# cvlab-stonybrook/s-volsdf

Hardware: AMD Instinct MI355X
Metric: rendered rays/sec (1024-ray batch, 128 samples) (higher is better)
Workload: dtype f32 (every product, forward and backward, as three fp16 MFMA products of two-piece fp16 operands with f32 accumulate; activation blocks hold both pieces: float32 accuracy class)

## Files before the change

include/svolsdf_hip.h:

```cpp
#ifndef SVOLSDF_HIP_H
#define SVOLSDF_HIP_H

#include <stddef.h>
#include <stdint.h>

#ifdef __cplusplus
extern "C" {
#endif

int svs_version(void);
const char* svs_last_error_string(void);

int svs_set_deterministic(int on);
int svs_get_deterministic(void);

int svs_rays_from_uv(const float* uv, const float* pose, const float* intrinsics, int n_rays, float* ray_dirs,
                     float* cam_loc, float* depth_scale, void* hip_stream);

int svs_eikonal_points(const float* uniform_points, const float* cam_loc, const float* z_eik, const float* ray_dirs,
                       int n_rays, float* points, void* hip_stream);
int svs_stage_in(const void* pinned_host, void* device, size_t bytes, void* hip_stream);
int svs_split_last(const float* z, int n_rays, int n, float* head, float* last, void* hip_stream);

enum { SVS_MMA_F32 = 0, SVS_MMA_F16X2 = 1, SVS_MMA_F16X2_HALF = 2 };
// ... 74 lines not shown
  const float* absmax;
  const float *rec0, *rec1;
} svs_wgrad_job;
int svs_wgrad_multi(const svs_wgrad_job* jobs, int n_jobs, int precision, void* hip_stream);
int svs_wgrad(const float* a0, const float* b0, long long sa0, long long sb0, const float* a1, const float* b1,
              long long sa1, long long sb1, const float* b_extra, long long s_extra, int n_points, int precision,
              const float* absmax, const float* rec0, const float* rec1, float* dW, int ldw, float* db, void* hip_stream);

size_t svs_block_bytes(int n_points, int blocks_per_tile);
size_t svs_rgb_zbuf_bytes(int n_points);
size_t svs_sdf_ubuf_bytes(int n_points);
size_t svs_sdf_gbuf_bytes(int n_points);
int svs_rgb_bwd(int n_points, const float* d_rgb, const float* rgb, const float* rbuf, const float* stream, int precision,
                float* zbuf, float* feat_bar, float* d_normals, float* absmax, void* hip_stream);
int svs_sdf_bwd_a(const float* points, int n_points, const float* cam, int cam_stride, const float* dirs, const float* z,
                  int S, int n_rays, const float* d_grad, const unsigned char* clamp_mask, const float* hbuf,
                  const float* gbuf, const float* stream, int precision, float* ubuf, float* a2buf, float* pebuf,
                  float* absmax, void* hip_stream);
int svs_sdf_bwd_b(int n_points, const float* d_sdf, const unsigned char* clamp_mask, const float* feat_bar,
                  int n_feat_points, const float* hbuf, const float* gbuf, const float* a2buf, const float* ubuf,
                  const float* stream, int precision, float* abuf, float* sbar_out, float* absmax, void* hip_stream);
int svs_lin8_row0_grad(const float* hbuf, const float* ubuf, const float* sbar, int n_points, int precision, float* out257,
                       void* hip_stream);
int svs_unpack_wgrad(const float* dWk, const float* dbk, int ldw, int map, int rows, int cols, int row_off,
                     const float* weight_v, const float* weight_g, const float* row0, float* grad_v, float* grad_g,
                     float* grad_b, void* hip_stream);
typedef struct svs_unpack_job {
  const float *dWk, *dbk;
  int ldw, map, rows, cols, row_off;
  const float *weight_v, *weight_g, *row0;
  float *grad_v, *grad_g, *grad_b;
} svs_unpack_job;
int svs_unpack_wgrad_multi(const svs_unpack_job* jobs, int n_jobs, void* hip_stream);

size_t svs_adam_workspace_bytes(void);
int svs_clip_guard_adam(float* params, float* grads, float* exp_avg, float* exp_avg_sq, long long n, int step,
                        int* step_counter, double max_norm, double lr, double beta1, double beta2, double eps,
                        void* workspace, float* info, void* hip_stream);

int svs_cost_lookup(const float* xyz, const float* cam, const float* dirs, const float* z, int S, int n_points,
                    int n_views, int same_view, int inverse_depth, float img_w, float img_h, const float* view_params,
                    const float* const* cost, const float* const* z_near, const float* const* z_far, const int* dims,
                    float* pj, float* pi, unsigned char* valid, const int* same_view_dev, void* hip_stream);

int svs_loss(int n_rays, int n_samples, int n_eik, const float* rgb_values, const float* rgb_target,
             const float* grad_theta, const float* weights, const float* pi, const float* pj, const float* depth_values,
// ... 108 lines not shown
```

s-volsdf_amd/csrc/svs_mlp_bwd.hip:

```cpp
#include "svs_mlp_dev.h"
#include "svs_mlp_bwd_args.h"
#include "svs_ticket.h"

namespace svs {
namespace mlp {


__global__ __launch_bounds__(kThreads, 1) void rgb_bwd_kernel(RgbBwdArgs a) {
  extern __shared__ __attribute__((aligned(16))) unsigned char smem[];
  Stream st;
  st.g = a.stream; st.buf = reinterpret_cast<f32x4*>(smem); st.cur = 1;
  const int lane = threadIdx.x & 63, half = lane >> 5, wave = threadIdx.x >> 6;
  const int wtile = blockIdx.x * kWaves + wave;
  const int p = wtile * kTilePts + (lane & 31);
  const bool livep = p < a.P;
  const int pc = livep ? p : a.P - 1;
  const size_t LS = block_stride();
  const float* rb = a.rbuf + (size_t)wtile * kBlockF;
  float* zb = a.zbuf + (size_t)wtile * kBlockF;

  st.prefetch<kW4TF4>();
  float dz[3];
#pragma unroll
  for (int c = 0; c < 3; ++c) {
// ... 403 lines not shown
  SdfBwdAArgs a;
  const bool h2 = is_h2(precision);
  if (n_points < 0 || n_rays < 0 || (n_points == 0 && n_rays == 0) || (n_points > 0 && !points) ||
      (n_rays > 0 && !(cam && dirs && z && S > 0)) || !d_grad || !hbuf || (!h2 && !gbuf) || !stream || !ubuf || (!h2 && !a2buf) ||
      !pebuf) {
    set_error("svs_sdf_bwd_a: null/invalid argument"); return SVS_EINVAL;
  }
  a.src.pts = points; a.src.cam = cam; a.src.dirs = dirs; a.src.z = z; a.src.cam_stride = cam_stride;
  a.src.S = S > 0 ? S : 1; a.src.n_ray = n_rays * (S > 0 ? S : 0); a.src.P = a.src.n_ray + n_points;
  a.d_grad = d_grad; a.clamp_mask = clamp_mask; a.hbuf = hbuf; a.gbuf = gbuf;
  a.stream = reinterpret_cast<const f32x4*>(stream); a.ubuf = ubuf; a.a2buf = a2buf; a.pebuf = pebuf;
  a.absmax = absmax;
  if (h2) {
    if (!absmax) { set_error("svs_sdf_bwd_a: fp16x2 needs absmax"); return SVS_EINVAL; }
    return launch_sdf_bwd_a_h2(a, precision == kFmtF16x2, (hipStream_t)hip_stream);
  }
  if (precision != kFmtF32) { set_error("svs_sdf_bwd_a: unknown precision %d", precision); return SVS_EINVAL; }
  static int once = set_lds_b(sdf_bwd_a_kernel, kLdsBytes, "svs_sdf_bwd_a");
  if (once) return once;
  sdf_bwd_a_kernel<<<(a.src.P + kWgPts - 1) / kWgPts, kThreads, kLdsBytes, (hipStream_t)hip_stream>>>(a);
  return check_launch("svs_sdf_bwd_a");
}

int svs_sdf_bwd_b(int n_points, const float* d_sdf, const unsigned char* clamp_mask, const float* feat_bar,
                  int n_feat_points, const float* hbuf, const float* gbuf, const float* a2buf, const float* ubuf,
                  const float* stream, int precision, float* abuf, float* sbar_out, float* absmax, void* hip_stream) {
  const bool h2 = is_h2(precision);
  if (!hbuf || !gbuf || (h2 ? !ubuf : !a2buf) || !stream || !abuf || !sbar_out || n_points <= 0 || n_feat_points % 32) {
    set_error("svs_sdf_bwd_b: null/invalid argument (n_feat_points must be a multiple of 32)"); return SVS_EINVAL;
  }
  SdfBwdBArgs a{n_points, d_sdf, clamp_mask, feat_bar, n_feat_points / 32, hbuf, gbuf, a2buf, ubuf,
                reinterpret_cast<const f32x4*>(stream) + kSdfTrainPassBF4, abuf, sbar_out, absmax,
                gbuf + 7 * (size_t)tiles_of(n_points) * kBlockF, (size_t)kBlockF};
  if (h2) {
    if (!absmax) { set_error("svs_sdf_bwd_b: fp16x2 needs absmax"); return SVS_EINVAL; }
    return launch_sdf_bwd_b_h2(a, precision == kFmtF16x2, (hipStream_t)hip_stream);
  }
  if (precision != kFmtF32) { set_error("svs_sdf_bwd_b: unknown precision %d", precision); return SVS_EINVAL; }
  static int once = set_lds_b(sdf_bwd_b_kernel, kLdsBytes, "svs_sdf_bwd_b");
  if (once) return once;
  sdf_bwd_b_kernel<<<(n_points + kWgPts - 1) / kWgPts, kThreads, kLdsBytes, (hipStream_t)hip_stream>>>(a);
  return check_launch("svs_sdf_bwd_b");
}

int svs_lin8_row0_grad(const float* hbuf, const float* ubuf, const float* sbar, int n_points, int precision, float* out257,
                       void* hip_stream) {
  if (!hbuf || !sbar || !out257 || n_points <= 0) { set_error("svs_lin8_row0_grad: bad argument"); return SVS_EINVAL; }
  if (is_h2(precision)) return launch_lin8_row0_h2(hbuf, ubuf, sbar, n_points, tiles_of(n_points), out257, precision == kFmtF16x2, (hipStream_t)hip_stream);
  if (precision != kFmtF32) { set_error("svs_lin8_row0_grad: unknown precision %d", precision); return SVS_EINVAL; }
  const int n_tiles = (n_points + 31) / 32;
  const int grid = n_tiles < 1024 ? n_tiles : 1024;
  const det::Ticket ticket{det::take_slots(1), 0u, (unsigned)grid};
  lin8_row0_kernel<<<grid, 256, 0, (hipStream_t)hip_stream>>>(hbuf, ubuf, sbar, n_tiles, tiles_of(n_points), n_points, out257, ticket);
  return check_launch("svs_lin8_row0_grad");
}

int svs_unpack_wgrad(const float* dWk, const float* dbk, int ldw, int map, int rows, int cols, int row_off,
                     const float* weight_v, const float* weight_g, const float* row0, float* grad_v, float* grad_g,
                     float* grad_b, void* hip_stream) {
  if (!dWk || !weight_v || !grad_v || rows < 1 || cols < 1 || map < 0 || map > 4 || (weight_g && !grad_g)) {
    set_error("svs_unpack_wgrad: bad argument"); return SVS_EINVAL;
  }
  UnpackArgs a{dWk, dbk, ldw, map, rows, cols, row_off, weight_v, weight_g, grad_v, grad_g, grad_b, row0};
  unpack_wgrad_kernel<<<(rows + 3) / 4, 256, 0, (hipStream_t)hip_stream>>>(a);
  return check_launch("svs_unpack_wgrad");
// ... 23 lines not shown
```

s-volsdf_amd/csrc/svs_mlp_bwd_args.h:

```cpp
#pragma once
#include "svs_mlp_dev.h"

namespace svs {
namespace mlp {

struct RgbBwdArgs {
  int P;
  const float* d_rgb;
  const float* rgb;
  const float* rbuf;
  const f32x4* stream;
  float* zbuf;
  float* feat_bar;
  float* d_normals;
  float* absmax;
};
constexpr int kRbufFb = 4 * kBlockF + 1024;

struct SdfBwdAArgs {
  PointSrc src;
  const float* d_grad;
  const unsigned char* clamp_mask;
  const float* hbuf;
  const float* gbuf;
  const f32x4* stream;
  float* ubuf;
  float* a2buf;
  float* pebuf;
  float* absmax;
};

struct SdfBwdBArgs {
  int P;
  const float* d_sdf;
  const unsigned char* clamp_mask;
  const float* feat_bar;
  int n_feat_tiles;
  const float* hbuf; const float* gbuf;
  const float* a2buf;
  const float* ubuf;
  const f32x4* stream;
  float* abuf;
  float* sbar_out;
  float* absmax;
  const float* w0; size_t w0_stride;
  int reverse = 0;
};
int launch_bg_bwd_b_h2(const SdfBwdBArgs& a, bool gp, hipStream_t s);

int launch_rgb_bwd_h2(const RgbBwdArgs& a, bool gp, hipStream_t s);
int launch_lin8_row0_h2(const float* hbuf, const float* ubuf, const float* sbar, int n_points, int n_tiles_pad, float* out257,
                        bool gp, hipStream_t s);
int launch_sdf_bwd_a_h2(const SdfBwdAArgs& a, bool gp, hipStream_t s);
int launch_sdf_bwd_b_h2(const SdfBwdBArgs& a, bool gp, hipStream_t s);

}
}
```

s-volsdf_amd/csrc/svs_mlp_bwd_h2.hip:

```cpp
#include "svs_mlp_h2_dev.h"
#include "svs_mlp_host.h"
#include "svs_mlp_bwd_args.h"
#include "svs_mlp_h2_trunk.h"
#include "svs_mlp_bwd_h2_dev.h"
#include "svs_ticket.h"
#include <cstdlib>

namespace svs {
namespace mlp {

template <bool GP>
struct RgbBwdEpi {
  f32x16 prev;
  TilePieces r;
  float v8[8];
  Pieces2* out;
  float* zblk;
  PointScale* ps;
  int lane;
  __device__ __forceinline__ void b(int tp, int rr) {
    float v = prev[rr] * ps->inv_in;
    v = hi_at(r, rr) > 0.0f ? v : 0.0f;
    pin(v);
    ps->track(v);
// ... 321 lines not shown
      st.advance();
    }
    ep.all(7);
    ep.end();
    ps.next();
  }
  for (int l = 1; l < 7; ++l) {
    PassAEpi<true, GP> ep;
    ep.out = &pa; ep.ublk = ub + (size_t)(l + 1) * LS; ep.urec = urec(l + 1);
    ep.ps = &ps; ep.splice = splice; ep.lane = lane; ep.half = half; ep.l3 = l == 3;
    pass_a_layer_h2<true, false, GP>(st, pb, ep, hb + (size_t)l * LS, lane);
#pragma unroll
    for (int s = 0; s < 16; ++s) { pb.h[s] = pa.h[s]; pb.m[s] = pa.m[s]; }
  }
  {
    PassAEpi<false, GP> ep;
    ep.out = nullptr; ep.ublk = ub + (size_t)8 * LS; ep.urec = urec(8);
    ep.ps = &ps; ep.splice = splice; ep.lane = lane; ep.half = half; ep.l3 = false;
    pass_a_layer_h2<false, true, GP>(st, pb, ep, hb + (size_t)7 * LS, lane);
  }
  publish_max(a.absmax, ps.gmax);
}

template <bool FIRST, bool SPLIT, typename Net, bool A2, bool GP>
struct PassBEpi {
  static constexpr bool kG = A2 || FIRST;
  f32x16 prev;
  TilePieces h, u, g;
  float v, s1, q;
  float v8[8];
  f16x8 ap[2], aq[2];
  Pieces2* out;
  float* ablk;
  float* arec;
  PointScale* ps;
  float sbar, u_inv100;
  int lane, half;
  bool l4;
  __device__ __forceinline__ void a(int r) {
    v = prev[r] * ps->inv_in;
    float e = __builtin_amdgcn_exp2f(grad_times<GP>(h, r, -100.0f * 1.44269504088896341f));
    if (A2) e = __builtin_fminf(e, 0.99999994f);
    s1 = 1.0f - e;
    if (A2) q = e * u_inv100;
    pin(v); pin(s1);
    if (A2) pin(q);
  }
  template <bool LATE = false>
  __device__ __forceinline__ void b(int tp, int r) {
    float o = v * s1;
    if (A2) {
      const float gg = grad_mix<GP>(g, r);
      const float t = grad_times<GP>(u, r, gg);
      o = __builtin_fmaf(t, q * __builtin_amdgcn_rcpf(s1), o);
      if (FIRST) o = __builtin_fmaf(sbar, gg, o);
    } else if (FIRST) {
      o = __builtin_fmaf(sbar, grad_mix<GP>(g, r), o);
    }
    if (l4 && tp > Net::kSpliceTile) o = 0.0f;
    if (l4 && tp == Net::kSpliceTile) {
      const bool z0 = rho(r) >= Net::kSpliceLocal, z1 = rho(r) + 4 >= Net::kSpliceLocal;
      if (z0 || z1) { if (half ? z1 : z0) o = 0.0f; }
    }
    pin(o);
    ps->track(o);
    v8[r & 7] = o * ps->s_out;
    if ((r & 7) == 7) {
      const int k = 2 * tp + (r >> 3), q2 = r >> 3;
      if (SPLIT) {
        split8(v8, out->h[k], out->m[k]);
        pin(out->h[k], out->m[k]);
        ap[q2] = out->h[k];
        if (GP) aq[q2] = out->m[k];
      } else if (GP) {
        split8(v8, ap[q2], aq[q2]);
      } else {
        ap[q2] = hi8(v8, 1.0f);
      }
      if (!LATE) store_grad<GP>(ablk, k, lane, ap[q2], aq[q2]);
    }
  }
  __device__ __forceinline__ void store_slot(int tp, int s) {
    if (s == 9) store_grad<GP>(ablk, 2 * tp, lane, ap[0], aq[0]);
    if (s == 15) store_grad<GP>(ablk, 2 * tp + 1, lane, ap[1], aq[1]);
  }
  __device__ __forceinline__ void all(int tp) {
#pragma unroll
    for (int r = 0; r < 16; ++r) { a(r); b(tp, r); }
  }
};

template <bool FIRST, bool SPLIT, bool LAST_STAGE, typename Net, bool A2, bool GP>
__device__ __forceinline__ void pass_b_stage_h2(Stream& st, const Pieces2& in, PassBEpi<FIRST, SPLIT, Net, A2, GP>& ep, const float* hblk,
                                                const float* ublk, const float* urec, const float* gblk, float next_floor, int lane) {
  constexpr bool kG = A2 || FIRST;
  store_record(ep.arec, lane, ep.ps->s_out, 0.0f);
  ep.u_inv100 = A2 ? 100.0f * PointScale::inv_pow2(load_scale(urec, lane)) : 0.0f;
  TilePieces hnext, unext, gnext;
  load_tile_grad<GP>(hblk, 0, lane, hnext);
  if (A2) load_tile_grad<GP>(ublk, 0, lane, unext);
  if (kG) load_tile_grad<GP>(gblk, 0, lane, gnext);
  constexpr int kPer = GP ? 4 : 2;
  constexpr int kLoads = kPer * (1 + (A2 ? 1 : 0) + (kG ? 1 : 0));
  constexpr int kStores = GP ? 4 : 2;
#pragma unroll
  for (int t = 0; t < 8; ++t) {
    const TilePieces hcur = hnext, ucur = unext, gcur = gnext;
    auto side = [&](int s) {
      if (t == 7) return;
      if (s == 10) hnext.h[0] = load_piece(hblk, 2 * (t + 1), lane);
      if (s == 11) hnext.h[1] = load_piece(hblk, 2 * (t + 1) + 1, lane);
      if (A2 && s == 12) unext.h[0] = load_piece(ublk, 2 * (t + 1), lane);
      if (A2 && s == 13) unext.h[1] = load_piece(ublk, 2 * (t + 1) + 1, lane);
      if (kG && s == 14) gnext.h[0] = load_piece(gblk, 2 * (t + 1), lane);
      if (kG && s == 15) gnext.h[1] = load_piece(gblk, 2 * (t + 1) + 1, lane);
      if (GP) {
// ... 5 lines not shown
        if (kG && s == 15) gnext.m[1] = load_piece(gblk, 2 * (t + 1) + 1, lane, 1);
      }
    };
    const bool fetch = !(LAST_STAGE && t == 7);
    f32x16 acc;
    if (!fetch) acc = tile_mma_h2<16>(st.cur_buf(), in, lane, [&](int s) { ep.a(s); }, [&](int s) { ep.b(t - 1, s); });
    else if (t == 0) acc = tile_mma_h2_pf<16, kChunkF4>(st, in, lane, NoEpi(), NoEpi(), side);
    else acc = tile_mma_h2_pf<16, kChunkF4>(st, in, lane, [&](int s) { ep.a(s); },
                                            [&](int s) { ep.template b<true>(t - 1, s); ep.store_slot(t - 1, s); }, side);
    ep.prev = acc; ep.h = hcur;
    if (A2) ep.u = ucur;
    if (kG) ep.g = gcur;
    if (fetch) {
      if (t == 0) st.advance_keep<kLoads>();
      else if (t < 7) st.advance_keep<kLoads + kStores>();
      else st.advance_keep<kStores>();
    }
  }
  ep.all(7);
  ep.ps->floor_m = next_floor;
  ep.ps->next();
}

template <typename Net, bool A2, bool GP>
__global__ __launch_bounds__(kThreads, 1) void sdf_bwd_b_h2_kernel(SdfBwdBArgs a) {
  extern __shared__ __attribute__((aligned(16))) unsigned char smem[];
  Stream st;
  st.g = a.stream; st.buf = reinterpret_cast<f32x4*>(smem); st.cur = 1;
  const int lane = threadIdx.x & 63, half = lane >> 5, wave = threadIdx.x >> 6;
  const int bx = a.reverse ? (int)(gridDim.x - 1 - blockIdx.x) : (int)blockIdx.x;
  const int wtile = bx * kWaves + wave;
  const int p = wtile * kTilePts + (lane & 31);
  const int pc = p < a.P ? p : a.P - 1;
  st.prefetch<kChunkF4>();
  float sbar = (a.d_sdf && p < a.P) ? a.d_sdf[pc] : 0.0f;
  if (a.clamp_mask && a.clamp_mask[pc]) sbar = 0.0f;
  if (half == 0 && a.sbar_out) a.sbar_out[p] = sbar;
  const size_t LS = block_stride();
  const float* hb = a.hbuf + (size_t)wtile * kBlockF;
  const float* gb = A2 ? a.gbuf + (size_t)wtile * kBlockF : a.w0 + (size_t)wtile * a.w0_stride - 7 * LS;
  const float* ub = A2 ? a.ubuf + (size_t)wtile * kBlockF : nullptr;
  float* ab = a.abuf + (size_t)wtile * kBlockF;
  const size_t T = (size_t)gridDim.x * kWaves;
  auto arec = [&](int l) { return record_ptr(a.abuf, 8, T, l, wtile); };
  auto urec = [&](int l) { return A2 ? record_ptr(a.ubuf, 9, T, l, wtile) : nullptr; };
  const float asb = __builtin_fabsf(sbar);
  auto floor_of = [&](int l) {
// ... 2 lines not shown
  const bool has_f = a.feat_bar && wtile < a.n_feat_tiles;
  PointScale ps;
  Pieces2 pa, pb;
  {
    const float fl = floor_of(7);
    if (has_f) {
      const float* fb = a.feat_bar + (size_t)wtile * kBlockF;
      const float* frec = record_ptr(a.feat_bar, 1, (size_t)((a.n_feat_tiles + kWaves - 1) / kWaves * kWaves), 0, wtile);
#pragma unroll
      for (int k = 0; k < 16; ++k) {
        pa.h[k] = load_piece(fb, k, lane);
        pa.m[k] = GP ? load_piece(fb, k, lane, 1) : (f16x8)(_Float16)0.0f;
      }
      ps.start_stored(load_scale(frec, lane), load_max(frec, lane), fl);
    } else {
#pragma unroll
      for (int k = 0; k < 16; ++k) { pa.h[k] = (f16x8)(_Float16)0.0f; pa.m[k] = (f16x8)(_Float16)0.0f; }
      ps.start(0.0f, fl);
    }
    ps.gmax = 0.0f;
  }
  st.advance();
  {
    PassBEpi<true, true, Net, A2, GP> ep;
    ep.out = &pb; ep.ablk = ab + 7 * LS; ep.arec = arec(7); ep.ps = &ps; ep.sbar = sbar; ep.lane = lane; ep.half = half; ep.l4 = false;
    pass_b_stage_h2<true, true, false, Net, A2, GP>(st, pa, ep, hb + 7 * LS, A2 ? ub + 8 * LS : nullptr, urec(8), gb + 7 * LS,
                                                    floor_of(6), lane);
  }
  for (int l = 7; l >= 2; --l) {
    PassBEpi<false, true, Net, A2, GP> ep;
    ep.out = &pa; ep.ablk = ab + (size_t)(l - 1) * LS; ep.arec = arec(l - 1); ep.ps = &ps; ep.sbar = 0.0f; ep.lane = lane; ep.half = half;
    ep.l4 = l == 4;
    pass_b_stage_h2<false, true, false, Net, A2, GP>(st, pb, ep, hb + (size_t)(l - 1) * LS, A2 ? ub + (size_t)l * LS : nullptr, urec(l),
                                                     A2 ? gb + (size_t)(l - 1) * LS : nullptr, floor_of(l >= 2 ? l - 2 : 0), lane);
#pragma unroll
    for (int s = 0; s < 16; ++s) { pb.h[s] = pa.h[s]; pb.m[s] = pa.m[s]; }
  }
  {
    PassBEpi<false, false, Net, A2, GP> ep;
    ep.out = nullptr; ep.ablk = ab; ep.arec = arec(0); ep.ps = &ps; ep.sbar = 0.0f; ep.lane = lane; ep.half = half; ep.l4 = false;
    pass_b_stage_h2<false, false, true, Net, A2, GP>(st, pb, ep, hb, A2 ? ub + LS : nullptr, urec(1), A2 ? gb : nullptr, asb, lane);
  }
  publish_max(a.absmax, ps.gmax);
}

template <bool GP>
__global__ __launch_bounds__(256) void lin8_row0_h2_kernel(const float* __restrict__ hbuf, const float* __restrict__ ubuf,
                                                           const float* __restrict__ sbar, int n_tiles, int n_tiles_pad, int P,
                                                           float* __restrict__ out, det::Ticket ticket) {
  __shared__ float red[4][32][65];
  const int lane = threadIdx.x & 63, quarter = threadIdx.x >> 6;
  float acc[32];
#pragma unroll
  for (int i = 0; i < 32; ++i) acc[i] = 0.0f;
  float bsum = 0.0f;
  for (int t = blockIdx.x; t < n_tiles; t += gridDim.x) {
    const int p = t * 32 + (lane & 31);
    const float sb = p < P ? sbar[p] : 0.0f;
    const float* h = hbuf + ((size_t)7 * n_tiles_pad + t) * kBlockF;
    f16x8 hh[4], hm[4], uh[4], um[4];
    float us = 0.0f;
#pragma unroll
    for (int k = 0; k < 4; ++k) { hh[k] = load_piece(h, 4 * quarter + k, lane, 0); hm[k] = load_piece(h, 4 * quarter + k, lane, 1); }
    if (ubuf) {
      const float* u = ubuf + ((size_t)8 * n_tiles_pad + t) * kBlockF;
#pragma unroll
// ... 41 lines not shown
  else lin8_row0_h2_kernel<false><<<grid, 256, 0, s>>>(hbuf, ubuf, sbar, n_tiles, n_tiles_pad, n_points, out257, ticket);
  return check_launch("svs_lin8_row0_grad");
}

int launch_rgb_bwd_h2(const RgbBwdArgs& a, bool gp, hipStream_t s) {
  static int once = set_lds(rgb_bwd_h2_kernel<true>, kLdsBytes, "svs_rgb_bwd") | set_lds(rgb_bwd_h2_kernel<false>, kLdsBytes, "svs_rgb_bwd");
  if (once) return once;
  const int grid = (a.P + kWgPts - 1) / kWgPts;
  if (gp) rgb_bwd_h2_kernel<true><<<grid, kThreads, kLdsBytes, s>>>(a);
  else rgb_bwd_h2_kernel<false><<<grid, kThreads, kLdsBytes, s>>>(a);
  return check_launch("svs_rgb_bwd");
}
int launch_sdf_bwd_a_h2(const SdfBwdAArgs& a, bool gp, hipStream_t s) {
  constexpr int lds = kLdsBytes + kSpliceF * kThreads * (int)sizeof(float);
  static int once = set_lds(sdf_bwd_a_h2_kernel<true>, lds, "svs_sdf_bwd_a") | set_lds(sdf_bwd_a_h2_kernel<false>, lds, "svs_sdf_bwd_a");
  if (once) return once;
  const int grid = (a.src.P + kWgPts - 1) / kWgPts;
  if (gp) sdf_bwd_a_h2_kernel<true><<<grid, kThreads, lds, s>>>(a);
  else sdf_bwd_a_h2_kernel<false><<<grid, kThreads, lds, s>>>(a);
  return check_launch("svs_sdf_bwd_a");
}
int launch_sdf_bwd_b_h2(const SdfBwdBArgs& a_in, bool gp, hipStream_t s) {
  static int once = set_lds(sdf_bwd_b_h2_kernel<NetFg, true, true>, kLdsBytes, "svs_sdf_bwd_b") |
                    set_lds(sdf_bwd_b_h2_kernel<NetFg, true, false>, kLdsBytes, "svs_sdf_bwd_b");
  if (once) return once;
  static const int reverse_env = [] { const char* e = getenv("SVS_BWD_B_REVERSE"); return e ? atoi(e) : 0; }();
  SdfBwdBArgs a = a_in;
  a.reverse = reverse_env;
  const int grid = (a.P + kWgPts - 1) / kWgPts;
  if (gp) sdf_bwd_b_h2_kernel<NetFg, true, true><<<grid, kThreads, kLdsBytes, s>>>(a);
  else sdf_bwd_b_h2_kernel<NetFg, true, false><<<grid, kThreads, kLdsBytes, s>>>(a);
  return check_launch("svs_sdf_bwd_b");
}
int launch_bg_bwd_b_h2(const SdfBwdBArgs& a, bool gp, hipStream_t s) {
  static int once = set_lds(sdf_bwd_b_h2_kernel<NetBg, false, true>, kLdsBytes, "svs_bg_sdf_bwd") |
                    set_lds(sdf_bwd_b_h2_kernel<NetBg, false, false>, kLdsBytes, "svs_bg_sdf_bwd");
  if (once) return once;
  const int grid = (a.P + kWgPts - 1) / kWgPts;
  if (gp) sdf_bwd_b_h2_kernel<NetBg, false, true><<<grid, kThreads, kLdsBytes, s>>>(a);
  else sdf_bwd_b_h2_kernel<NetBg, false, false><<<grid, kThreads, kLdsBytes, s>>>(a);
  return check_launch("svs_bg_sdf_bwd");
}

}
}
```

s-volsdf_amd/svs_hip/lib.py:

```python
import ctypes
import os
from ctypes import POINTER, c_char_p, c_double, c_float, c_int, c_longlong, c_size_t, c_void_p

_HERE = os.path.dirname(os.path.abspath(__file__))
LIB_PATH = os.environ.get("SVS_LIB_PATH") or os.path.join(os.path.dirname(_HERE), "lib", "libsvolsdf_hip.so")

_lib = None


class SvsError(RuntimeError):
    pass


_P = c_void_p
_PP = POINTER(c_void_p)

class WGradJob(ctypes.Structure):
    _fields_ = [("a0", ctypes.c_void_p), ("b0", ctypes.c_void_p), ("sa0", ctypes.c_longlong), ("sb0", ctypes.c_longlong),
                ("a1", ctypes.c_void_p), ("b1", ctypes.c_void_p), ("sa1", ctypes.c_longlong), ("sb1", ctypes.c_longlong),
                ("b_extra", ctypes.c_void_p), ("s_extra", ctypes.c_longlong),
                ("n_points", ctypes.c_int), ("ldw", ctypes.c_int),
                ("dW", ctypes.c_void_p), ("db", ctypes.c_void_p), ("absmax", ctypes.c_void_p),
                ("rec0", ctypes.c_void_p), ("rec1", ctypes.c_void_p)]

# ... 12 lines not shown
    "svs_last_error_string": (c_char_p, []),
    "svs_rays_from_uv": (c_int, [_P, _P, _P, c_int, _P, _P, _P, _P]),
    "svs_stream_bytes": (c_size_t, [c_int]),
    "svs_pack_stream": (c_int, [c_int, c_int, _PP, _PP, _PP, _P, _P, _P]),
    "svs_pack_workspace_bytes": (c_size_t, []),
    "svs_sdf_vals": (c_int, [_P, c_int, _P, c_int, _P, _P, c_int, c_int, _P, c_int, c_float, c_float, c_int, _P, _P,
                             c_int, c_int, _P]),
    "svs_sdf_hbuf_bytes": (c_size_t, [c_int]),
    "svs_sdf_gbuf_bytes": (c_size_t, [c_int]),
    "svs_feat_tiles_bytes": (c_size_t, [c_int]),
    "svs_sdf_outputs": (c_int, [_P, c_int, _P, c_int, _P, _P, c_int, c_int, _P, c_int, c_float, c_float, c_int, _P, _P,
                                _P, _P, _P, _P, _P]),
    "svs_tiles_to_rows": (c_int, [_P, c_int, c_int, _P, _P]),
    "svs_rgb_eval": (c_int, [_P, c_int, _P, c_int, _P, _P, c_int, c_int, _P, _P, c_int, _P, _P, c_int, _P, _P, _P]),
    "svs_rgb_rbuf_bytes": (c_size_t, [c_int]),
    "svs_block_bytes": (c_size_t, [c_int, c_int]),
    "svs_rgb_zbuf_bytes": (c_size_t, [c_int]),
    "svs_sdf_ubuf_bytes": (c_size_t, [c_int]),
    "svs_rgb_bwd": (c_int, [c_int, _P, _P, _P, _P, c_int, _P, _P, _P, _P, _P]),
    "svs_sdf_bwd_a": (c_int, [_P, c_int, _P, c_int, _P, _P, c_int, c_int, _P, _P, _P, _P, _P, c_int, _P, _P, _P,
                              _P, _P]),
    "svs_sdf_bwd_b": (c_int, [c_int, _P, _P, _P, c_int, _P, _P, _P, _P, _P, c_int, _P, _P, _P, _P]),
    "svs_lin8_row0_grad": (c_int, [_P, _P, _P, c_int, c_int, _P, _P]),
    "svs_unpack_wgrad": (c_int, [_P, _P, c_int, c_int, c_int, c_int, c_int, _P, _P, _P, _P, _P, _P, _P]),
    "svs_unpack_wgrad_multi": (c_int, [_P, c_int, _P]),
    "svs_sampler_ctl_bytes": (c_size_t, [c_int, c_int]),
    "svs_sampler_ctl_stride": (c_int, []),
    "svs_sampler_cap": (c_int, []),
    "svs_sampler_max_new": (c_int, []),
    "svs_sampler_init": (c_int, [_P, c_int, _P, c_int, c_int, c_float, c_float, c_int, c_float, _P, c_float, c_int,
                                 _P, _P, _P, _P, c_int, _P, _P]),
    "svs_sampler_round": (c_int, [c_int, c_int, c_int, c_int, c_int, c_int, c_int, _P, c_float, c_float, c_int, c_float,
                                  c_float, _P, _P, _P, _P, _P, _P, _P, c_int, _P, _P, _P, _P, _P, _P, _P, _P, _P, _P]),
    "svs_composite": (c_int, [c_int, c_int, _P, _P, _P, _P, _P, _P, c_float, _P, _P, _P, _P, _P, _P]),
    "svs_composite_bwd": (c_int, [c_int, c_int, _P, _P, _P, _P, _P, c_float, _P, _P, _P, _P, _P, _P, _P, _P]),
    "svs_wgrad": (c_int, [_P, _P, ctypes.c_longlong, ctypes.c_longlong, _P, _P, ctypes.c_longlong, ctypes.c_longlong,
                          _P, ctypes.c_longlong, c_int, c_int, _P, _P, _P, _P, c_int, _P, _P]),
    "svs_wgrad_multi": (c_int, [_P, c_int, c_int, _P]),
    "svs_bg_points": (c_int, [_P, c_int, _P, c_int, c_int, _P, c_float, _P, _P, _P, _P]),
    "svs_bg_sdf_eval": (c_int, [_P, c_int, _P, c_int, _P, _P, _P, _P, _P, _P]),
    "svs_bg_rgb_bwd": (c_int, [c_int, _P, _P, _P, _P, c_int, _P, _P, _P, _P]),
    "svs_bg_sdf_bwd": (c_int, [c_int, _P, _P, _P, _P, _P, c_int, _P, _P, _P, _P]),
    "svs_bg_rbuf_bytes": (c_size_t, [c_int]),
    "svs_bg_rgb_eval": (c_int, [c_int, _P, c_int, _P, _P, c_int, _P, _P, _P]),
    "svs_composite_bg_bwd": (c_int, [c_int, c_int, c_int, _P, _P, _P, _P, _P, _P, c_float, _P, _P, _P, _P, _P, _P, _P, _P,
                                     _P, _P, _P, _P, _P, _P, _P]),
# ... 110 lines not shown
```

s-volsdf_amd/svs_hip/profiling.py:

```python
import torch

from . import lib as _lib


class LaunchTimer:

    def __init__(self, names):
        self.names = list(names)
        self.events = {n: [] for n in self.names}
        self._orig = {}
        self.meta = {n: [] for n in self.names}

    def __enter__(self):
        L = _lib.load()
        for n in self.names:
            fn = getattr(L, n)
            self._orig[n] = fn
            setattr(L, n, self._wrap(n, fn))
        return self

    def _wrap(self, name, fn):
        def call(*args):
            e0, e1 = torch.cuda.Event(enable_timing=True), torch.cuda.Event(enable_timing=True)
            e0.record()
            rc = fn(*args)
            e1.record()
            self.events[name].append((e0, e1))
            self.meta[name].append(args)
            return rc
        return call

    def __exit__(self, *exc):
        L = _lib.load()
        for n, fn in self._orig.items():
            setattr(L, n, fn)
        return False

    def times_ms(self, name):
        return [a.elapsed_time(b) for a, b in self.events[name]]
```

s-volsdf_amd/svs_hip/train.py:

```python
import ctypes
import os

import torch

from . import lib as _lib
from .ops import _f32, _ptr, _ptr_array, _stream, default_precision, is_h2, F16X2, F16X2_HALF

KBLOCK = 128 * 64
KREC = 64


def block_stride(n_points):
    return ((n_points + 127) // 128) * 4 * KBLOCK
LDW = 288


def n_tiles_padded(n_points):
    return ((n_points + 127) // 128) * 4


def record_off(n_points, n_blocks, block):
    T = n_tiles_padded(n_points)
    return n_blocks * T * KBLOCK + block * T * KREC

# ... 78 lines not shown

    def __init__(self, device, streams=None, accum=None):
        self.dev = device
        self.streams = streams or TrainStreams(device)
        self.accum = accum or WGradAccum(device)
        self._n = None
        self._side = None
        self._job_cache = {}
        self.time_wgrad = False
        self.timer_events = None

    def _alloc(self, n_total, n_main):
        if self._n == (n_total, n_main):
            return
        L = _lib.load()
        z = lambda nbytes: torch.zeros(nbytes // 4, device=self.dev)
        self.zbuf = z(L.svs_rgb_zbuf_bytes(n_main))
        self.feat_bar = z(L.svs_block_bytes(n_main, 1))
        self.ubuf = z(L.svs_sdf_ubuf_bytes(n_total))
        self.a2buf = z(L.svs_block_bytes(n_total, 8)) if not is_h2(self.streams.precision) else None
        self.abuf = z(L.svs_block_bytes(n_total, 8))
        self.pebuf = z(L.svs_block_bytes(n_total, 1))
        self.sbar = z(L.svs_block_bytes(n_total, 1) // (128 * 2))
        self.d_sdf_full = torch.zeros(n_total, device=self.dev)
        self.d_grad_full = torch.zeros(n_total, 3, device=self.dev)
        self._n = (n_total, n_main)

    def _cache_jobs(self, key, jobs):
        if len(self._job_cache) >= 64:
            self._job_cache.clear()
        arr = (_lib.WGradJob * len(jobs))(*jobs)
        hit = self._job_cache[key] = (ctypes.cast(arr, ctypes.c_void_p), len(jobs), arr)
        return hit[:2]

    def sdf_grad_out(self, n_total, n_main):
        self._alloc(n_total, n_main)
        return self.d_sdf_full[:n_main].view(n_main, 1)

    def grad_extra_out(self, n_total, n_main):
        self._alloc(n_total, n_main)
        return self.d_grad_full[n_main:]

    def accumulate(self, keep, d_rgb, d_sdf, d_grad_extra, wait=True, side=True, defer_wgrad=False, extra=None):
        L = _lib.load()
        src = keep["src"]
        n_total, n_main = src.n, keep["rgb"].shape[0]
# ... 69 lines not shown
            for l in range(1, 5):
                jobs.append(job(9 + l, n_main, 1, _off(self.zbuf, l * LSm), KBLOCK, _off(rbuf, (l - 1) * LSm), KBLOCK,
                                rec0=zrec(l)))
            return jobs

        deferred = None
        if defer_wgrad:
            ev_rgb = torch.cuda.Event(); ev_rgb.record(main)
            deferred = dict(rgb=dict(jobs=job_list(rkey, rgb_jobs), key=rkey), ev_rgb=ev_rgb)
            join = None
        else:
            fork = torch.cuda.Event(); fork.record(main)
            with torch.cuda.stream(side_stream):
                if side:
                    side_stream.wait_event(fork)
                if extra is not None:
                    side_stream.wait_event(extra["ev_rgb"])
                wgrad_multi(job_array(rkey, job_list(rkey, rgb_jobs), extra["rgb"] if extra else None))
                join = torch.cuda.Event(); join.record(side_stream)
        st = _stream()
        _lib.check(L.svs_sdf_bwd_a(*src.args(), _ptr(d_grad), _ptr(mask), _ptr(hbuf), _ptr(gbuf), _ptr(S.sdf), prec,
                                   _ptr(self.ubuf), _ptr(self.a2buf), _ptr(self.pebuf),
                                   _ptr(acc.absmax) if h2 else None, st), "svs_sdf_bwd_a")
        _lib.check(L.svs_sdf_bwd_b(n_total, _ptr(d_sdf_full), _ptr(mask), _ptr(self.feat_bar), n_main, _ptr(hbuf),
                                   _ptr(gbuf), _ptr(self.a2buf), _ptr(self.ubuf), _ptr(S.sdf), prec, _ptr(self.abuf),
                                   _ptr(self.sbar), _ptr(acc.absmax) if h2 else None, st),
                   "svs_sdf_bwd_b")
        _lib.check(L.svs_lin8_row0_grad(_ptr(hbuf), _ptr(self.ubuf), _ptr(self.sbar), n_total, prec, _ptr(acc.row0),
                                        _stream()), "svs_lin8_row0_grad")
        ev = self.timer_events = ([torch.cuda.Event(enable_timing=True) for _ in range(2)] if self.time_wgrad else None)
        if ev:
            ev[0].record()
        skey = ("sdf", n_total, n_main, prec, self.abuf.data_ptr(), self.ubuf.data_ptr(), self.pebuf.data_ptr(),
                hbuf.data_ptr(), gbuf.data_ptr(), self.feat_bar.data_ptr(), acc.dWk.data_ptr())

        def sdf_jobs():
            arec = lambda l: _off(self.abuf, record_off(n_total, 8, l))
            urec = lambda l: _off(self.ubuf, record_off(n_total, 9, l))
            second = lambda l: dict(a1=_off(gbuf, l * LS), sa1=KBLOCK, b1=_off(self.ubuf, l * LS), sb1=KBLOCK, rec1=urec(l))
            jobs = [job(0, n_total, 0, _off(self.abuf, 0), KBLOCK, _ptr(self.pebuf), KBLOCK, rec0=arec(0), **second(0))]
            for l in range(1, 8):
                jobs.append(job(l, n_total, 0, _off(self.abuf, l * LS), KBLOCK, _off(hbuf, (l - 1) * LS), KBLOCK, rec0=arec(l),
                                **second(l)))
            jobs.append(job(8, n_main, 2, _ptr(self.feat_bar), KBLOCK, _off(hbuf, 7 * LS), KBLOCK,
                            rec0=_off(self.feat_bar, record_off(n_main, 1, 0))))
            return jobs

        if defer_wgrad:
            deferred["sdf"] = dict(jobs=job_list(skey, sdf_jobs), key=skey)
            deferred["ev_all"] = torch.cuda.Event(); deferred["ev_all"].record(main)
            deferred["hold"] = self._hold = (d_grad, d_sdf_full, d_normals, d_rgb)
            return deferred
# ... 133 lines not shown
```

Baseline: 292,300.

## Fuse lin8 row-0 gradient reduction into SDF backward pass B epilogue

Computes the per-point contributions to the layer-8 row-0 weight gradient inside the fp16x2 sdf_bwd_b kernel epilogue. It uses DPP lane folds and an LDS reduction, writes per-workgroup partials to a workspace, and sums them with a small follow-up kernel. This replaces the separate svs_lin8_row0_grad pass, which re-read hbuf, ubuf and sbar. It costs extra LDS per workgroup, extra registers in the epilogue, and a new partial-sum kernel with atomics.

After: 295,400, median of 6. About the same (+1.1%).

```diff
diff --git a/include/svolsdf_hip.h b/include/svolsdf_hip.h
--- a/include/svolsdf_hip.h
+++ b/include/svolsdf_hip.h
@@ -120,6 +120,11 @@
                   const float* stream, int precision, float* abuf, float* sbar_out, float* absmax, void* hip_stream);
 int svs_lin8_row0_grad(const float* hbuf, const float* ubuf, const float* sbar, int n_points, int precision, float* out257,
                        void* hip_stream);
+size_t svs_sdf_row0_ws_bytes(int n_points);
+int svs_sdf_bwd_b_row0(int n_points, const float* d_sdf, const unsigned char* clamp_mask, const float* feat_bar,
+                       int n_feat_points, const float* hbuf, const float* gbuf, const float* a2buf, const float* ubuf,
+                       const float* stream, int precision, float* abuf, float* sbar_out, float* absmax, float* row0_ws,
+                       float* out257, void* hip_stream);
 int svs_unpack_wgrad(const float* dWk, const float* dbk, int ldw, int map, int rows, int cols, int row_off,
                      const float* weight_v, const float* weight_g, const float* row0, float* grad_v, float* grad_g,
                      float* grad_b, void* hip_stream);
diff --git a/s-volsdf_amd/csrc/svs_mlp_bwd.hip b/s-volsdf_amd/csrc/svs_mlp_bwd.hip
--- a/s-volsdf_amd/csrc/svs_mlp_bwd.hip
+++ b/s-volsdf_amd/csrc/svs_mlp_bwd.hip
@@ -449,25 +449,62 @@
   return check_launch("svs_sdf_bwd_a");
 }
 
+int svs_lin8_row0_grad(const float* hbuf, const float* ubuf, const float* sbar, int n_points, int precision, float* out257,
+                       void* hip_stream);
+
+}
+
+namespace {
+int sdf_bwd_b(int n_points, const float* d_sdf, const unsigned char* clamp_mask, const float* feat_bar, int n_feat_points,
+              const float* hbuf, const float* gbuf, const float* a2buf, const float* ubuf, const float* stream, int precision,
+              float* abuf, float* sbar_out, float* absmax, float* row0_ws, float* out257, hipStream_t hs) {
+  const bool h2 = is_h2(precision);
+  if (!hbuf || !gbuf || (h2 ? !ubuf : !a2buf) || !stream || !abuf || !sbar_out || n_points <= 0 || n_feat_points % 32) {
+    set_error("svs_sdf_bwd_b: null/invalid argument (n_feat_points must be a multiple of 32)"); return SVS_EINVAL;
+  }
+  const bool fused = out257 && precision == kFmtF16x2;
+  if (fused && !row0_ws) { set_error("svs_sdf_bwd_b_row0: no workspace"); return SVS_EINVAL; }
+  SdfBwdBArgs a{n_points, d_sdf, clamp_mask, feat_bar, n_feat_points / 32, hbuf, gbuf, a2buf, ubuf,
+                reinterpret_cast<const f32x4*>(stream) + kSdfTrainPassBF4, abuf, sbar_out, absmax,
+                gbuf + 7 * (size_t)tiles_of(n_points) * kBlockF, (size_t)kBlockF};
+  a.row0_part = fused ? row0_ws : nullptr;
+  int rc;
+  if (h2) {
+    if (!absmax) { set_error("svs_sdf_bwd_b: fp16x2 needs absmax"); return SVS_EINVAL; }
+    rc = launch_sdf_bwd_b_h2(a, precision == kFmtF16x2, hs);
+  } else {
+    if (precision != kFmtF32) { set_error("svs_sdf_bwd_b: unknown precision %d", precision); return SVS_EINVAL; }
+    static int once = set_lds_b(sdf_bwd_b_kernel, kLdsBytes, "svs_sdf_bwd_b");
+    if (once) return once;
+    sdf_bwd_b_kernel<<<(n_points + kWgPts - 1) / kWgPts, kThreads, kLdsBytes, hs>>>(a);
+    rc = check_launch("svs_sdf_bwd_b");
+  }
+  if (rc || !out257) return rc;
+  if (fused) return launch_lin8_row0_sum(row0_ws, (n_points + kWgPts - 1) / kWgPts, out257, hs);
+  return svs_lin8_row0_grad(hbuf, ubuf, sbar_out, n_points, precision, out257, hs);
+}
+}
+
+extern "C" {
+
 int svs_sdf_bwd_b(int n_points, const float* d_sdf, const unsigned char* clamp_mask, const float* feat_bar,
                   int n_feat_points, const float* hbuf, const float* gbuf, const float* a2buf, const float* ubuf,
                   const float* stream, int precision, float* abuf, float* sbar_out, float* absmax, void* hip_stream) {
-  const bool h2 = is_h2(precision);
-  if (!hbuf || !gbuf || (h2 ? !ubuf : !a2buf) || !stream || !abuf || !sbar_out || n_points <= 0 || n_feat_points % 32) {
-    set_error("svs_sdf_bwd_b: null/invalid argument (n_feat_points must be a multiple of 32)"); return SVS_EINVAL;
-  }
-  SdfBwdBArgs a{n_points, d_sdf, clamp_mask, feat_bar, n_feat_points / 32, hbuf, gbuf, a2buf, ubuf,
-                reinterpret_cast<const f32x4*>(stream) + kSdfTrainPassBF4, abuf, sbar_out, absmax,
-                gbuf + 7 * (size_t)tiles_of(n_points) * kBlockF, (size_t)kBlockF};
-  if (h2) {
-    if (!absmax) { set_error("svs_sdf_bwd_b: fp16x2 needs absmax"); return SVS_EINVAL; }
-    return launch_sdf_bwd_b_h2(a, precision == kFmtF16x2, (hipStream_t)hip_stream);
-  }
-  if (precision != kFmtF32) { set_error("svs_sdf_bwd_b: unknown precision %d", precision); return SVS_EINVAL; }
-  static int once = set_lds_b(sdf_bwd_b_kernel, kLdsBytes, "svs_sdf_bwd_b");
-  if (once) return once;
-  sdf_bwd_b_kernel<<<(n_points + kWgPts - 1) / kWgPts, kThreads, kLdsBytes, (hipStream_t)hip_stream>>>(a);
-  return check_launch("svs_sdf_bwd_b");
+  return sdf_bwd_b(n_points, d_sdf, clamp_mask, feat_bar, n_feat_points, hbuf, gbuf, a2buf, ubuf, stream, precision, abuf,
+                   sbar_out, absmax, nullptr, nullptr, (hipStream_t)hip_stream);
+}
+
+size_t svs_sdf_row0_ws_bytes(int n_points) {
+  return (size_t)((n_points + kWgPts - 1) / kWgPts) * kRow0Pitch * sizeof(float);
+}
+
+int svs_sdf_bwd_b_row0(int n_points, const float* d_sdf, const unsigned char* clamp_mask, const float* feat_bar,
+                       int n_feat_points, const float* hbuf, const float* gbuf, const float* a2buf, const float* ubuf,
+                       const float* stream, int precision, float* abuf, float* sbar_out, float* absmax, float* row0_ws,
+                       float* out257, void* hip_stream) {
+  if (!out257) { set_error("svs_sdf_bwd_b_row0: out257 is required"); return SVS_EINVAL; }
+  return sdf_bwd_b(n_points, d_sdf, clamp_mask, feat_bar, n_feat_points, hbuf, gbuf, a2buf, ubuf, stream, precision, abuf,
+                   sbar_out, absmax, row0_ws, out257, (hipStream_t)hip_stream);
 }
 
 int svs_lin8_row0_grad(const float* hbuf, const float* ubuf, const float* sbar, int n_points, int precision, float* out257,
diff --git a/s-volsdf_amd/csrc/svs_mlp_bwd_args.h b/s-volsdf_amd/csrc/svs_mlp_bwd_args.h
--- a/s-volsdf_amd/csrc/svs_mlp_bwd_args.h
+++ b/s-volsdf_amd/csrc/svs_mlp_bwd_args.h
@@ -45,7 +45,9 @@
   float* absmax;
   const float* w0; size_t w0_stride;
   int reverse = 0;
+  float* row0_part = nullptr;
 };
+constexpr int kRow0Pitch = 260;
 int launch_bg_bwd_b_h2(const SdfBwdBArgs& a, bool gp, hipStream_t s);
 
 int launch_rgb_bwd_h2(const RgbBwdArgs& a, bool gp, hipStream_t s);
@@ -53,6 +55,7 @@
                         bool gp, hipStream_t s);
 int launch_sdf_bwd_a_h2(const SdfBwdAArgs& a, bool gp, hipStream_t s);
 int launch_sdf_bwd_b_h2(const SdfBwdBArgs& a, bool gp, hipStream_t s);
+int launch_lin8_row0_sum(const float* part, int n_part, float* out257, hipStream_t s);
 
 }
 }
diff --git a/s-volsdf_amd/csrc/svs_mlp_bwd_h2.hip b/s-volsdf_amd/csrc/svs_mlp_bwd_h2.hip
--- a/s-volsdf_amd/csrc/svs_mlp_bwd_h2.hip
+++ b/s-volsdf_amd/csrc/svs_mlp_bwd_h2.hip
@@ -367,7 +367,21 @@
   publish_max(a.absmax, ps.gmax);
 }
 
-template <bool FIRST, bool SPLIT, typename Net, bool A2, bool GP>
+constexpr int kRow0RedBytes = kWaves * 8 * 64 * 4;
+constexpr int kRow0LdsBytes = kRow0RedBytes + kWaves * 4;
+__device__ __forceinline__ unsigned lds_byte_addr(const void* p) {
+  return (unsigned)(unsigned long long)(const __attribute__((address_space(3))) void*)p;
+}
+template <int N, int CTRL>
+__device__ __forceinline__ void r0_fold(float* v, bool up) {
+#pragma unroll
+  for (int i = 0; i < N; ++i) {
+    const float keep = up ? v[i + N] : v[i], send = up ? v[i] : v[i + N];
+    v[i] = keep + __builtin_bit_cast(float, __builtin_amdgcn_mov_dpp(__builtin_bit_cast(int, send), CTRL, 0xf, 0xf, true));
+  }
+}
+
+template <bool FIRST, bool SPLIT, typename Net, bool A2, bool GP, bool R0 = false>
 struct PassBEpi {
   static constexpr bool kG = A2 || FIRST;
   f32x16 prev;
@@ -382,6 +396,19 @@
   float sbar, u_inv100;
   int lane, half;
   bool l4;
+  float r0_us;
+  unsigned r0_lds;
+  __device__ __forceinline__ void row0(int tp) {
+    float x[16];
+#pragma unroll
+    for (int r = 0; r < 16; ++r) x[r] = grad_times<GP>(h, r, sbar) + grad_times<GP>(u, r, r0_us);
+    const int j = lane & 15;
+    r0_fold<8, 0x141>(x, (j >> 2) & 1);
+    r0_fold<4, 0x128>(x, (j >> 3) & 1);
+    r0_fold<2, 0x4e>(x, (j >> 1) & 1);
+    r0_fold<1, 0xb1>(x, j & 1);
+    asm volatile("ds_write_b32 %0, %1" :: "v"(r0_lds + 256u * tp), "v"(x[0]) : "memory");
+  }
   __device__ __forceinline__ void a(int r) {
     v = prev[r] * ps->inv_in;
     float e = __builtin_amdgcn_exp2f(grad_times<GP>(h, r, -100.0f * 1.44269504088896341f));
@@ -424,6 +451,7 @@
       }
       if (!LATE) store_grad<GP>(ablk, k, lane, ap[q2], aq[q2]);
     }
+    if (R0 && r == 15) row0(tp);
   }
   __device__ __forceinline__ void store_slot(int tp, int s) {
     if (s == 9) store_grad<GP>(ablk, 2 * tp, lane, ap[0], aq[0]);
@@ -435,8 +463,8 @@
   }
 };
 
-template <bool FIRST, bool SPLIT, bool LAST_STAGE, typename Net, bool A2, bool GP>
-__device__ __forceinline__ void pass_b_stage_h2(Stream& st, const Pieces2& in, PassBEpi<FIRST, SPLIT, Net, A2, GP>& ep, const float* hblk,
+template <bool FIRST, bool SPLIT, bool LAST_STAGE, typename Net, bool A2, bool GP, bool R0 = false>
+__device__ __forceinline__ void pass_b_stage_h2(Stream& st, const Pieces2& in, PassBEpi<FIRST, SPLIT, Net, A2, GP, R0>& ep, const float* hblk,
                                                 const float* ublk, const float* urec, const float* gblk, float next_floor, int lane) {
   constexpr bool kG = A2 || FIRST;
   store_record(ep.arec, lane, ep.ps->s_out, 0.0f);
@@ -488,7 +516,7 @@
   ep.ps->next();
 }
 
-template <typename Net, bool A2, bool GP>
+template <typename Net, bool A2, bool GP, bool R0 = false>
 __global__ __launch_bounds__(kThreads, 1) void sdf_bwd_b_h2_kernel(SdfBwdBArgs a) {
   extern __shared__ __attribute__((aligned(16))) unsigned char smem[];
   Stream st;
@@ -537,9 +565,13 @@
   }
   st.advance();
   {
-    PassBEpi<true, true, Net, A2, GP> ep;
+    PassBEpi<true, true, Net, A2, GP, R0> ep;
     ep.out = &pb; ep.ablk = ab + 7 * LS; ep.arec = arec(7); ep.ps = &ps; ep.sbar = sbar; ep.lane = lane; ep.half = half; ep.l4 = false;
-    pass_b_stage_h2<true, true, false, Net, A2, GP>(st, pa, ep, hb + 7 * LS, A2 ? ub + 8 * LS : nullptr, urec(8), gb + 7 * LS,
+    if (R0) {
+      ep.r0_us = p < a.P ? PointScale::inv_pow2(load_scale(urec(8), lane)) : 0.0f;
+      ep.r0_lds = lds_byte_addr(smem + kLdsBytes) + 2048u * wave + 4u * lane;
+    }
+    pass_b_stage_h2<true, true, false, Net, A2, GP, R0>(st, pa, ep, hb + 7 * LS, A2 ? ub + 8 * LS : nullptr, urec(8), gb + 7 * LS,
                                                     floor_of(6), lane);
   }
   for (int l = 7; l >= 2; --l) {
@@ -557,6 +589,25 @@
     pass_b_stage_h2<false, false, true, Net, A2, GP>(st, pb, ep, hb, A2 ? ub + LS : nullptr, urec(1), A2 ? gb : nullptr, asb, lane);
   }
   publish_max(a.absmax, ps.gmax);
+  if (R0) {
+    const float* red = reinterpret_cast<const float*>(smem + kLdsBytes);
+    float* sbw = reinterpret_cast<float*>(smem + kLdsBytes + kRow0RedBytes);
+    float sb = half == 0 ? sbar : 0.0f;
+#pragma unroll
+    for (int d = 1; d < 32; d <<= 1) sb += __shfl_xor(sb, d);
+    if (lane == 0) sbw[wave] = sb;
+    __syncthreads();
+    const int f = threadIdx.x, tp = f >> 5, hf = (f >> 2) & 1, r = 4 * ((f & 31) >> 3) + (f & 3);
+    const int j = (r & 1) + 2 * ((r >> 1) & 1) + 4 * (r >> 3) + 8 * ((r >> 2) & 1);
+    float v = 0.0f;
+#pragma unroll
+    for (int w = 0; w < kWaves; ++w)
+#pragma unroll
+      for (int q = 0; q < 2; ++q) v += red[512 * w + 64 * tp + 16 * (2 * hf + q) + j];
+    float* part = a.row0_part + (size_t)bx * kRow0Pitch;
+    part[f] = v;
+    if (f == 0) part[256] = ((sbw[0] + sbw[1]) + sbw[2]) + sbw[3];
+  }
 }
 
 template <bool GP>
@@ -644,15 +695,37 @@
 }
 int launch_sdf_bwd_b_h2(const SdfBwdBArgs& a_in, bool gp, hipStream_t s) {
   static int once = set_lds(sdf_bwd_b_h2_kernel<NetFg, true, true>, kLdsBytes, "svs_sdf_bwd_b") |
-                    set_lds(sdf_bwd_b_h2_kernel<NetFg, true, false>, kLdsBytes, "svs_sdf_bwd_b");
+                    set_lds(sdf_bwd_b_h2_kernel<NetFg, true, false>, kLdsBytes, "svs_sdf_bwd_b") |
+                    set_lds(sdf_bwd_b_h2_kernel<NetFg, true, true, true>, kLdsBytes + kRow0LdsBytes, "svs_sdf_bwd_b");
   if (once) return once;
   static const int reverse_env = [] { const char* e = getenv("SVS_BWD_B_REVERSE"); return e ? atoi(e) : 0; }();
   SdfBwdBArgs a = a_in;
   a.reverse = reverse_env;
   const int grid = (a.P + kWgPts - 1) / kWgPts;
-  if (gp) sdf_bwd_b_h2_kernel<NetFg, true, true><<<grid, kThreads, kLdsBytes, s>>>(a);
+  if (gp && a.row0_part) sdf_bwd_b_h2_kernel<NetFg, true, true, true><<<grid, kThreads, kLdsBytes + kRow0LdsBytes, s>>>(a);
+  else if (gp) sdf_bwd_b_h2_kernel<NetFg, true, true><<<grid, kThreads, kLdsBytes, s>>>(a);
   else sdf_bwd_b_h2_kernel<NetFg, true, false><<<grid, kThreads, kLdsBytes, s>>>(a);
   return check_launch("svs_sdf_bwd_b");
+}
+
+__global__ __launch_bounds__(256) void lin8_row0_sum_kernel(const float* __restrict__ part, int n_part, float* __restrict__ out) {
+  __shared__ f32x4 red[256];
+  const int tid = threadIdx.x, c4 = blockIdx.x;
+  f32x4 v = (f32x4)(0.0f);
+  for (int w = tid; w < n_part; w += 256) v += reinterpret_cast<const f32x4*>(part + (size_t)w * kRow0Pitch)[c4];
+  red[tid] = v;
+  __syncthreads();
+#pragma unroll
+  for (int k = 128; k > 0; k >>= 1) {
+    if (tid < k) red[tid] += red[tid + k];
+    __syncthreads();
+  }
+  if (tid < 4 && 4 * c4 + tid < 257) atomicAdd(&out[4 * c4 + tid], red[0][tid]);
+}
+
+int launch_lin8_row0_sum(const float* part, int n_part, float* out257, hipStream_t s) {
+  lin8_row0_sum_kernel<<<kRow0Pitch / 4, 256, 0, s>>>(part, n_part, out257);
+  return check_launch("svs_sdf_bwd_b_row0");
 }
 int launch_bg_bwd_b_h2(const SdfBwdBArgs& a, bool gp, hipStream_t s) {
   static int once = set_lds(sdf_bwd_b_h2_kernel<NetBg, false, true>, kLdsBytes, "svs_bg_sdf_bwd") |
diff --git a/s-volsdf_amd/svs_hip/lib.py b/s-volsdf_amd/svs_hip/lib.py
--- a/s-volsdf_amd/svs_hip/lib.py
+++ b/s-volsdf_amd/svs_hip/lib.py
@@ -58,6 +58,8 @@
                               _P, _P]),
     "svs_sdf_bwd_b": (c_int, [c_int, _P, _P, _P, c_int, _P, _P, _P, _P, _P, c_int, _P, _P, _P, _P]),
     "svs_lin8_row0_grad": (c_int, [_P, _P, _P, c_int, c_int, _P, _P]),
+    "svs_sdf_row0_ws_bytes": (c_size_t, [c_int]),
+    "svs_sdf_bwd_b_row0": (c_int, [c_int, _P, _P, _P, c_int, _P, _P, _P, _P, _P, c_int, _P, _P, _P, _P, _P, _P]),
     "svs_unpack_wgrad": (c_int, [_P, _P, c_int, c_int, c_int, c_int, c_int, _P, _P, _P, _P, _P, _P, _P]),
     "svs_unpack_wgrad_multi": (c_int, [_P, c_int, _P]),
     "svs_sampler_ctl_bytes": (c_size_t, [c_int, c_int]),
diff --git a/s-volsdf_amd/svs_hip/profiling.py b/s-volsdf_amd/svs_hip/profiling.py
--- a/s-volsdf_amd/svs_hip/profiling.py
+++ b/s-volsdf_amd/svs_hip/profiling.py
@@ -11,12 +11,15 @@
         self._orig = {}
         self.meta = {n: [] for n in self.names}
 
+    ALIASES = {"svs_sdf_bwd_b": ("svs_sdf_bwd_b_row0",)}
+
     def __enter__(self):
         L = _lib.load()
         for n in self.names:
-            fn = getattr(L, n)
-            self._orig[n] = fn
-            setattr(L, n, self._wrap(n, fn))
+            for entry in (n,) + self.ALIASES.get(n, ()):
+                fn = getattr(L, entry)
+                self._orig[entry] = fn
+                setattr(L, entry, self._wrap(n, fn))
         return self
 
     def _wrap(self, name, fn):
diff --git a/s-volsdf_amd/svs_hip/train.py b/s-volsdf_amd/svs_hip/train.py
--- a/s-volsdf_amd/svs_hip/train.py
+++ b/s-volsdf_amd/svs_hip/train.py
@@ -124,6 +124,7 @@
         self.abuf = z(L.svs_block_bytes(n_total, 8))
         self.pebuf = z(L.svs_block_bytes(n_total, 1))
         self.sbar = z(L.svs_block_bytes(n_total, 1) // (128 * 2))
+        self.row0_ws = z(L.svs_sdf_row0_ws_bytes(n_total))
         self.d_sdf_full = torch.zeros(n_total, device=self.dev)
         self.d_grad_full = torch.zeros(n_total, 3, device=self.dev)
         self._n = (n_total, n_main)
@@ -239,12 +240,10 @@
         _lib.check(L.svs_sdf_bwd_a(*src.args(), _ptr(d_grad), _ptr(mask), _ptr(hbuf), _ptr(gbuf), _ptr(S.sdf), prec,
                                    _ptr(self.ubuf), _ptr(self.a2buf), _ptr(self.pebuf),
                                    _ptr(acc.absmax) if h2 else None, st), "svs_sdf_bwd_a")
-        _lib.check(L.svs_sdf_bwd_b(n_total, _ptr(d_sdf_full), _ptr(mask), _ptr(self.feat_bar), n_main, _ptr(hbuf),
-                                   _ptr(gbuf), _ptr(self.a2buf), _ptr(self.ubuf), _ptr(S.sdf), prec, _ptr(self.abuf),
-                                   _ptr(self.sbar), _ptr(acc.absmax) if h2 else None, st),
-                   "svs_sdf_bwd_b")
-        _lib.check(L.svs_lin8_row0_grad(_ptr(hbuf), _ptr(self.ubuf), _ptr(self.sbar), n_total, prec, _ptr(acc.row0),
-                                        _stream()), "svs_lin8_row0_grad")
+        _lib.check(L.svs_sdf_bwd_b_row0(n_total, _ptr(d_sdf_full), _ptr(mask), _ptr(self.feat_bar), n_main, _ptr(hbuf),
+                                        _ptr(gbuf), _ptr(self.a2buf), _ptr(self.ubuf), _ptr(S.sdf), prec, _ptr(self.abuf),
+                                        _ptr(self.sbar), _ptr(acc.absmax) if h2 else None, _ptr(self.row0_ws), _ptr(acc.row0),
+                                        st), "svs_sdf_bwd_b_row0")
         ev = self.timer_events = ([torch.cuda.Event(enable_timing=True) for _ in range(2)] if self.time_wgrad else None)
         if ev:
             ev[0].record()
```
